# aim-uofa/GenPercept

Hardware: AMD Instinct MI355X
Metric: images/sec at 768x768 bf16 (depth) (higher is better)
Workload: dtype bf16; 1 GPU; depth head, SD2.1 VAE-enc + UNet(t=1) + VAE-dec, 768x768, batch 4/GPU (BASELINE.json configs[1]); global_batch=4, resolution=768, parallelism=dp1 (batch-sharded, weights replicated, no data-path collective), weights=random-init SD2.1 architecture (865.9M + 83.7M params)

## Files before the change

genpercept_amd/csrc/attention.hip:

```cpp
#include <cstdlib>

#include "common.h"
#include "kernels.h"

GP_DEV int attn_off128(int row, int slot) { return row * 128 + ((slot ^ ((row >> 1) & 7)) << 4); }

#ifndef GP_FLASH_DEFER
#define GP_FLASH_DEFER 0.f
#endif
template <int NKB>
__global__ __launch_bounds__(256, 2) void flash_attn64_kernel(const h16_t* __restrict__ Q, const h16_t* __restrict__ K,
                                                            const h16_t* __restrict__ Vt, h16_t* __restrict__ O, int T, int heads, int ldq,
                                                            int ldk, int Tpad, int ldo) {
    constexpr int KEYS = 32 * NKB, KBYTES = KEYS * 128, NH = NKB / 2;
    constexpr int STAGE = 2 * KBYTES;
    extern __shared__ __attribute__((aligned(16))) char smem[];
    const int tid = threadIdx.x, lane = tid & 63;
    const int wave = __builtin_amdgcn_readfirstlane(tid >> 6);
    const int nqb = (T + 127) >> 7;
    const int sid = xcd_remap(blockIdx.x, gridDim.x);
    const int qb = sid % nqb, bh = sid / nqb;
    const int h = bh % heads, b = bh / heads;
    const int q0 = qb * 128 + wave * 32;
    const int l31 = lane & 31, hh = lane >> 5;

    const h16_t* Qb = Q + (long long)b * T * ldq + h * 64;
    const h16_t* Kb = K + (long long)b * T * ldk + h * 64;
    const h16_t* Vb = Vt + ((long long)b * heads + h) * 64 * Tpad;

    h16x8_t qf[4];
    {
        const int q = q0 + l31;
        const bool ok = q < T;
#pragma unroll
        for (int ks = 0; ks < 4; ++ks) {
            if (ok) qf[ks] = *(const h16x8_t*)(Qb + (long long)q * ldq + ks * 16 + hh * 8);
            else qf[ks] = h16x8_t{0, 0, 0, 0, 0, 0, 0, 0};
        }
    }

    const int chunk = (lane & 7) ^ ((wave * 4 + (lane >> 4)) & 7);
    const int nt = (T + KEYS - 1) / KEYS;
    const buf_rsrc_t k_rs = make_rsrc(Kb, (unsigned)(((long long)T - 1) * ldk * 2 + 128));
    const buf_rsrc_t v_rs = make_rsrc(Vb, (unsigned)(64ll * Tpad * 2));
    const unsigned k_lane = (unsigned)(((lane >> 3) & 3) + 8 * (lane >> 5)) * (unsigned)(ldk * 2) + chunk * 16;
    const unsigned v_lane = ((unsigned)(lane >> 3) * Tpad + chunk * 8) * 2;
    auto stage = [&](int buf, int kt) {
        char* sb = smem + buf * STAGE;
#pragma unroll
        for (int i = 0; i < NKB; ++i) {
            const int g = wave + 4 * i;
            blds16(k_rs, k_lane, (unsigned)(kt * KEYS + (g >> 1) * 16 + 4 * (g & 1)) * (unsigned)(ldk * 2), sb + g * 1024);
        }
#pragma unroll
        for (int hf = 0; hf < NH; ++hf)
#pragma unroll
            for (int i = 0; i < 2; ++i) {
                const int k0 = kt * KEYS + hf * 64;
                const unsigned so = k0 < Tpad ? (unsigned)((wave + 4 * i) * 8 * Tpad + k0) * 2u : 0xfffff000u;
                blds16(v_rs, v_lane, so, sb + KBYTES + hf * 8192 + (wave + 4 * i) * 1024);
            }
    };

    f32x16_t o_acc[2];
#pragma unroll
    for (int d = 0; d < 2; ++d)
#pragma unroll
        for (int r = 0; r < 16; ++r) o_acc[d][r] = 0.f;
    float m_run = -1e30f;
    float l_run = 0.f;
    const float sc = 0.125f * 1.44269504088896340736f;
    f32x16_t zero16;
#pragma unroll
    for (int r = 0; r < 16; ++r) zero16[r] = 0.f;
    int cur = 0;
    const unsigned smem_base = (unsigned)(unsigned long long)smem;

    auto tile = [&](int kt, auto maskc) __attribute__((always_inline)) {
        constexpr bool MASK = decltype(maskc)::value != 0;
        const unsigned sb = smem_base + cur * STAGE;
        f32x16_t s_acc[NKB];
#pragma unroll
        for (int kb = 0; kb < NKB; ++kb) {
            const int row = kb * 32 + l31;
#pragma unroll
            for (int ks = 0; ks < 4; ++ks) {
                const h16x8_t kf = lds_frag(sb + attn_off128(row, ks * 2 + hh), 0);
                s_acc[kb] = mfma_32x32x16(kf, qf[ks], ks == 0 ? zero16 : s_acc[kb]);
            }
        }
        if (MASK) {
            const int kbase = kt * KEYS + 8 * hh;
#pragma unroll
            for (int kb = 0; kb < NKB; ++kb)
#pragma unroll
                for (int r = 0; r < 16; ++r)
                    if (kbase + kb * 32 + (r & 7) + 16 * (r >> 3) >= T) s_acc[kb][r] = -1e30f;
        }
        float mx = s_acc[0][0];
#pragma unroll
        for (int kb = 0; kb < NKB; ++kb)
#pragma unroll
            for (int r = 0; r < 16; ++r) mx = fmaxf(mx, s_acc[kb][r]);
        mx = xor32_max(mx);
        if (__builtin_amdgcn_ballot_w64((mx - m_run) * sc > GP_FLASH_DEFER) != 0ull) {
            const float m_new = fmaxf(m_run, mx);
            const float alpha = __builtin_amdgcn_exp2f((m_run - m_new) * sc);
            m_run = m_new;
            l_run *= alpha;
#pragma unroll
            for (int d = 0; d < 2; ++d)
#pragma unroll
                for (int r = 0; r < 16; ++r) o_acc[d][r] *= alpha;
        }
        typedef float f32x2_t __attribute__((ext_vector_type(2)));
        const f32x2_t sc2 = {sc, sc}, nm2 = {-m_run * sc, -m_run * sc};
        f32x2_t rs2 = {0.f, 0.f};
#pragma unroll
        for (int kb = 0; kb < NKB; ++kb)
#pragma unroll
            for (int r = 0; r < 16; r += 2) {
                f32x2_t t = {s_acc[kb][r], s_acc[kb][r + 1]};
                t = __builtin_elementwise_fma(t, sc2, nm2);
                t.x = __builtin_amdgcn_exp2f(t.x);
                t.y = __builtin_amdgcn_exp2f(t.y);
                s_acc[kb][r] = t.x;
                s_acc[kb][r + 1] = t.y;
                rs2 += t;
            }
        l_run += rs2.x + rs2.y;
#pragma unroll
        for (int kb = 0; kb < NKB; ++kb)
#pragma unroll
            for (int j = 0; j < 2; ++j) {
                union { h16x8_t v; unsigned u[4]; } pf;
#pragma unroll
                for (int e = 0; e < 4; ++e) pf.u[e] = pack_h16x2_ns(s_acc[kb][8 * j + 2 * e], s_acc[kb][8 * j + 2 * e + 1]);
                const int slot = (kb & 1) * 4 + 2 * j + hh;
#pragma unroll
                for (int d = 0; d < 2; ++d) {
                    const h16x8_t vf = lds_frag(sb + KBYTES + (kb >> 1) * 8192 + attn_off128(d * 32 + l31, slot), 0);
                    o_acc[d] = mfma_32x32x16(vf, pf.v, o_acc[d]);
                }
            }
    };

#pragma unroll
    for (int s0 = 0; s0 < 1; ++s0)
        if (s0 < nt) stage(s0, s0);
    int nxt = 1;
    auto step = [&](int kt, auto maskc) __attribute__((always_inline)) {
        wait_vm<0>();
        __builtin_amdgcn_s_barrier();
        if (kt + 1 < nt) stage(nxt, kt + 1);
        tile(kt, maskc);
        cur = cur + 1 == 2 ? 0 : cur + 1;
        nxt = nxt + 1 == 2 ? 0 : nxt + 1;
    };
    const bool ragged = nt * KEYS > T;
    const int nfull = ragged ? nt - 1 : nt;
    for (int kt = 0; kt < nfull; ++kt) step(kt, IC<0>{});
    if (ragged) step(nt - 1, IC<1>{});
    l_run += __shfl_xor(l_run, 32);
    const float inv = 1.f / l_run;
    const int q = q0 + l31;
    if (q < T) {
        h16_t* ob = O + ((long long)b * T + q) * ldo + h * 64;
#pragma unroll
        for (int d = 0; d < 2; ++d)
#pragma unroll
            for (int g = 0; g < 4; ++g) {
                const uint2 pk = pack_h16x4(o_acc[d][4 * g] * inv, o_acc[d][4 * g + 1] * inv, o_acc[d][4 * g + 2] * inv, o_acc[d][4 * g + 3] * inv);
                *(uint2*)(ob + d * 32 + 8 * g + 4 * hh) = pk;
            }
    }
}

void launch_flash_attn64(const h16_t* q, const h16_t* k, const h16_t* vt, h16_t* out, int B, int T, int heads,
                         int ldq, int ldk, int Tpad, int ldo, hipStream_t s) {
    dim3 grid(((T + 127) / 128) * heads * B);
    hipLaunchKernelGGL(flash_attn64_kernel<2>, grid, dim3(256), 2 * 16384, s, q, k, vt, out, T, heads, ldq, ldk, Tpad, ldo);
}

__global__ __launch_bounds__(256, 2) void flash_attn64_split_kernel(const h16_t* __restrict__ QKhi, const h16_t* __restrict__ QKlo,
                                                                  const h16_t* __restrict__ Vthi, const h16_t* __restrict__ Vtlo,
                                                                  h16_t* __restrict__ O, int T, int heads, int ld, int Tpad) {
    constexpr int KEYS = 64, KBYTES = 8192, STAGE = 4 * KBYTES;
    extern __shared__ __attribute__((aligned(16))) char smem[];
    const int tid = threadIdx.x, lane = tid & 63;
    const int wave = __builtin_amdgcn_readfirstlane(tid >> 6);
    const int nqb = (T + 127) >> 7;
    const int sid = xcd_remap(blockIdx.x, gridDim.x);
    const int qb = sid % nqb, bh = sid / nqb;
    const int h = bh % heads, b = bh / heads;
    const int C = heads * 64;
    const int q0 = qb * 128 + wave * 32;
    const int l31 = lane & 31, hh = lane >> 5;

    const long long qoff = (long long)b * T * ld + h * 64;
    const long long voff = ((long long)b * heads + h) * 64 * Tpad;
    h16x8_t qh[4], ql[4];
    {
        const int q = q0 + l31;
        const bool ok = q < T;
#pragma unroll
        for (int ks = 0; ks < 4; ++ks) {
            if (ok) {
                qh[ks] = *(const h16x8_t*)(QKhi + qoff + (long long)q * ld + ks * 16 + hh * 8);
                ql[ks] = *(const h16x8_t*)(QKlo + qoff + (long long)q * ld + ks * 16 + hh * 8);
            } else {
                qh[ks] = ql[ks] = h16x8_t{0, 0, 0, 0, 0, 0, 0, 0};
            }
        }
    }
    const int chunk = (lane & 7) ^ ((wave * 4 + (lane >> 4)) & 7);
    const int nt = (T + KEYS - 1) / KEYS;
    const unsigned kbytes = (unsigned)(((long long)T - 1) * ld * 2 + 128);
    const buf_rsrc_t kh_rs = make_rsrc(QKhi + qoff + C, kbytes), kl_rs = make_rsrc(QKlo + qoff + C, kbytes);
    const buf_rsrc_t vh_rs = make_rsrc(Vthi + voff, (unsigned)(64ll * Tpad * 2)), vl_rs = make_rsrc(Vtlo + voff, (unsigned)(64ll * Tpad * 2));
    const unsigned k_lane = (unsigned)(((lane >> 3) & 3) + 8 * (lane >> 5)) * (unsigned)(ld * 2) + chunk * 16;
    const unsigned v_lane = ((unsigned)(lane >> 3) * Tpad + chunk * 8) * 2;
    auto stage = [&](int buf, int kt) {
        char* sb = smem + buf * STAGE;
#pragma unroll
        for (int i = 0; i < 2; ++i) {
            const int g = wave + 4 * i;
            const unsigned ko = (unsigned)(kt * KEYS + (g >> 1) * 16 + 4 * (g & 1)) * (unsigned)(ld * 2);
            blds16(kh_rs, k_lane, ko, sb + g * 1024);
            blds16(kl_rs, k_lane, ko, sb + KBYTES + g * 1024);
            const int k0 = kt * KEYS;
            const unsigned so = k0 < Tpad ? (unsigned)((wave + 4 * i) * 8 * Tpad + k0) * 2u : 0xfffff000u;
            blds16(vh_rs, v_lane, so, sb + 2 * KBYTES + g * 1024);
            blds16(vl_rs, v_lane, so, sb + 3 * KBYTES + g * 1024);
        }
    };
    f32x16_t o_acc[2];
#pragma unroll
    for (int d = 0; d < 2; ++d)
#pragma unroll
        for (int r = 0; r < 16; ++r) o_acc[d][r] = 0.f;
    float m_run = -1e30f, l_run = 0.f;
    const float sc = 0.125f * 1.44269504088896340736f;
    f32x16_t zero16;
#pragma unroll
    for (int r = 0; r < 16; ++r) zero16[r] = 0.f;
    int cur = 0;
    const unsigned smem_base = (unsigned)(unsigned long long)smem;

    auto tile = [&](int kt, auto maskc) __attribute__((always_inline)) {
        constexpr bool MASK = decltype(maskc)::value != 0;
        const unsigned sb = smem_base + cur * STAGE;
        f32x16_t s_acc[2];
#pragma unroll
        for (int kb = 0; kb < 2; ++kb) {
            const int row = kb * 32 + l31;
#pragma unroll
            for (int ks = 0; ks < 4; ++ks) {
                const h16x8_t kfh = lds_frag(sb + attn_off128(row, ks * 2 + hh), 0);
                const h16x8_t kfl = lds_frag(sb + KBYTES + attn_off128(row, ks * 2 + hh), 0);
                s_acc[kb] = mfma_32x32x16(kfl, qh[ks], ks == 0 ? zero16 : s_acc[kb]);
                s_acc[kb] = mfma_32x32x16(kfh, ql[ks], s_acc[kb]);
                s_acc[kb] = mfma_32x32x16(kfh, qh[ks], s_acc[kb]);
            }
        }
        if (MASK) {
            const int kbase = kt * KEYS + 8 * hh;
#pragma unroll
            for (int kb = 0; kb < 2; ++kb)
#pragma unroll
                for (int r = 0; r < 16; ++r)
                    if (kbase + kb * 32 + (r & 7) + 16 * (r >> 3) >= T) s_acc[kb][r] = -1e30f;
        }
        float mx = s_acc[0][0];
#pragma unroll
        for (int kb = 0; kb < 2; ++kb)
#pragma unroll
            for (int r = 0; r < 16; ++r) mx = fmaxf(mx, s_acc[kb][r]);
        mx = xor32_max(mx);
        if (__builtin_amdgcn_ballot_w64(mx > m_run) != 0ull) {
            const float m_new = fmaxf(m_run, mx);
            const float alpha = __builtin_amdgcn_exp2f((m_run - m_new) * sc);
            m_run = m_new;
            l_run *= alpha;
#pragma unroll
            for (int d = 0; d < 2; ++d)
#pragma unroll
                for (int r = 0; r < 16; ++r) o_acc[d][r] *= alpha;
        }
        const float nm = -m_run * sc;
        float rs = 0.f;
#pragma unroll
        for (int kb = 0; kb < 2; ++kb)
#pragma unroll
            for (int r = 0; r < 16; ++r) {
                const float t = __builtin_amdgcn_exp2f(__builtin_fmaf(s_acc[kb][r], sc, nm));
                s_acc[kb][r] = t;
                rs += t;
            }
        l_run += rs;
#pragma unroll
        for (int kb = 0; kb < 2; ++kb)
#pragma unroll
            for (int j = 0; j < 2; ++j) {
                union { h16x8_t v; unsigned u[4]; } ph, pl;
#pragma unroll
                for (int e = 0; e < 4; ++e) {
                    const float a = s_acc[kb][8 * j + 2 * e], c = s_acc[kb][8 * j + 2 * e + 1];
                    ph.u[e] = pack_h16x2_ns(a, c);
                    pl.u[e] = pack_h16x2_ns(a - h16_lo(ph.u[e]), c - h16_hi(ph.u[e]));
                }
                const int slot = kb * 4 + 2 * j + hh;
#pragma unroll
                for (int d = 0; d < 2; ++d) {
                    const h16x8_t vfh = lds_frag(sb + 2 * KBYTES + attn_off128(d * 32 + l31, slot), 0);
                    const h16x8_t vfl = lds_frag(sb + 3 * KBYTES + attn_off128(d * 32 + l31, slot), 0);
                    o_acc[d] = mfma_32x32x16(vfl, ph.v, o_acc[d]);
                    o_acc[d] = mfma_32x32x16(vfh, pl.v, o_acc[d]);
                    o_acc[d] = mfma_32x32x16(vfh, ph.v, o_acc[d]);
                }
            }
    };
    stage(0, 0);
    auto step = [&](int kt, auto maskc) __attribute__((always_inline)) {
        wait_vm<0>();
        __builtin_amdgcn_s_barrier();
        if (kt + 1 < nt) stage(cur ^ 1, kt + 1);
        tile(kt, maskc);
        cur ^= 1;
    };
    const bool ragged = nt * KEYS > T;
    const int nfull = ragged ? nt - 1 : nt;
    for (int kt = 0; kt < nfull; ++kt) step(kt, IC<0>{});
    if (ragged) step(nt - 1, IC<1>{});
    l_run += __shfl_xor(l_run, 32);
    const float inv = 1.f / l_run;
    const int q = q0 + l31;
    if (q < T) {
        h16_t* ob = O + ((long long)b * T + q) * 3 * C + h * 64;
#pragma unroll
        for (int d = 0; d < 2; ++d)
#pragma unroll
            for (int g = 0; g < 4; ++g) {
                const float v0 = o_acc[d][4 * g] * inv, v1 = o_acc[d][4 * g + 1] * inv, v2 = o_acc[d][4 * g + 2] * inv, v3 = o_acc[d][4 * g + 3] * inv;
                const unsigned h0 = pack_h16x2(v0, v1), h1 = pack_h16x2(v2, v3);
                const unsigned l0 = pack_h16x2(v0 - h16_lo(h0), v1 - h16_hi(h0)), l1 = pack_h16x2(v2 - h16_lo(h1), v3 - h16_hi(h1));
                const int c = d * 32 + 8 * g + 4 * hh;
                *(uint2*)(ob + c) = make_uint2(h0, h1);
                *(uint2*)(ob + C + c) = make_uint2(l0, l1);
                *(uint2*)(ob + 2 * C + c) = make_uint2(h0, h1);
            }
    }
}
void launch_flash_attn64_split(const h16_t* qk_hi, const h16_t* qk_lo, const h16_t* vt_hi, const h16_t* vt_lo, h16_t* out, int B, int T, int heads, int ld,
                               int Tpad, hipStream_t s) {
    static unsigned long long attr_mask = 0;
    gp_once_per_device(&attr_mask, [&] {
        (void)hipFuncSetAttribute((const void*)flash_attn64_split_kernel, hipFuncAttributeMaxDynamicSharedMemorySize, 2 * 32768);
    });
    dim3 grid(((T + 127) / 128) * heads * B);
    hipLaunchKernelGGL(flash_attn64_split_kernel, grid, dim3(256), 2 * 32768, s, qk_hi, qk_lo, vt_hi, vt_lo, out, T, heads, ld, Tpad);
}

constexpr int F5_KBYTES = 32 * 1024;
constexpr int F5_QV = 24;
constexpr int F5_RD = 6;
constexpr int F5_LDS = 4 * F5_KBYTES + 4 * (32 - F5_QV) * 1024;
typedef __attribute__((address_space(3))) h16x8_t* lds_frag_wptr;
GP_DEV float other_half(float v) {
    typedef unsigned u32x2p_t __attribute__((ext_vector_type(2)));
    const u32x2p_t r = __builtin_amdgcn_permlane32_swap(__float_as_uint(v), __float_as_uint(v), false, false);
    return (threadIdx.x & 32) ? __uint_as_float(r[0]) : __uint_as_float(r[1]);
}
GP_DEV int k512_off(int row, int slot) { return row * 1024 + ((slot ^ (row & 15)) << 4); }
GP_DEV int v512_off(int row, int slot) { return row * 64 + ((slot ^ ((row >> 2) & 3)) << 4); }
GP_DEV int pi23(int i) { return (i & ~12) | ((i & 4) << 1) | ((i & 8) >> 1); }

__global__ __launch_bounds__(256) void flash_attn512_kernel(const h16_t* __restrict__ Q, const h16_t* __restrict__ K,
                                                             const h16_t* __restrict__ Vt, h16_t* __restrict__ O,
                                                             float* __restrict__ part_o,
                                                             float* __restrict__ part_ml, int B, int T, int ldq, int ldk, int Tpad, int ldo,
                                                             float scale) {
    extern __shared__ __attribute__((aligned(16))) char smem[];
    const int tid = threadIdx.x, lane = tid & 63;
    const int wave = __builtin_amdgcn_readfirstlane(tid >> 6);
    const int l31 = lane & 31, hh = lane >> 5;
    const int nqb = (T + 127) >> 7, nblocks = B * nqb, G = gridDim.x;
    const int nt = (T + 31) >> 5;
    const int rounds = nblocks / G, L = nblocks - rounds * G, S = L ? G / L : 0;
    const int sid = xcd_remap(blockIdx.x, G);
    const unsigned smem_base = (unsigned)(unsigned long long)smem;
    const float sc = scale * 1.44269504088896340736f;
    f32x16_t zero16;
#pragma unroll
    for (int r = 0; r < 16; ++r) zero16[r] = 0.f;

    const int items = rounds + ((L && sid / S < L) ? 1 : 0);
    for (int it = 0; it < items; ++it) {
        const bool whole = it < rounds;
        const int part = whole ? 0 : sid % S;
        const int t0 = whole ? 0 : (int)((long long)nt * part / S), t1 = whole ? nt : (int)((long long)nt * (part + 1) / S);
        const int Li = (L % B == 0) ? L / B : 0;
        int b, qb;
        if (whole) {
            const int w = it * G + sid, per = nqb - Li;
            b = Li ? w / per : w / nqb;
            qb = Li ? w - b * per : w - b * nqb;
        } else {
            const int lb = sid / S;
            b = Li ? lb / Li : (rounds * G + lb) / nqb;
            qb = Li ? nqb - Li + (lb - b * Li) : rounds * G + lb - b * nqb;
        }
        const int q0 = qb * 128 + wave * 32;
        const h16_t* Qb = Q + (long long)b * T * ldq;
        const h16_t* Kb = K + (long long)b * T * ldk;
        const h16_t* Vb = Vt + (long long)b * 512 * Tpad;

        __syncthreads();
        h16x8_t qf[F5_QV];
        const unsigned q_lds = smem_base + 4 * F5_KBYTES + wave * ((32 - F5_QV) * 1024) + lane * 16;
        {
            const int q = q0 + l31;
            const bool ok = q < T;
#pragma unroll
            for (int ks = 0; ks < 32; ++ks) {
                h16x8_t v = h16x8_t{0, 0, 0, 0, 0, 0, 0, 0};
                if (ok) v = *(const h16x8_t*)(Qb + (long long)q * ldq + ks * 16 + hh * 8);
                if ((ks & 3) != 3) qf[3 * (ks >> 2) + (ks & 3)] = v;
                else *(lds_frag_wptr)(q_lds + (ks >> 2) * 1024) = v;
            }
            asm volatile("" ::"v"(qf[F5_QV - 1]));
        }
        const buf_rsrc_t k_rs = make_rsrc(Kb, (unsigned)((long long)T * ldk * 2));
        const buf_rsrc_t v_rs = make_rsrc(Vb, (unsigned)(512ll * Tpad * 2));
        unsigned koff[8];
#pragma unroll
        for (int n = 0; n < 8; ++n) koff[n] = (unsigned)(lane ^ ((wave & 1) * 8 + n)) << 4;
        const unsigned v_lane_off = ((unsigned)(lane >> 2) * Tpad + (((lane & 3) ^ ((lane >> 4) & 3)) << 3)) * 2;
        auto stage_piece = [&](int slot, int kt, int pc) __attribute__((always_inline)) {
            char* sb = smem + slot * F5_KBYTES;
            if (pc < 8) {
                const int i = wave * 8 + pc;
                const int key = min(kt * 32 + pi23(i), T - 1);
                blds16(k_rs, koff[pc & 7], (unsigned)key * (unsigned)(ldk * 2), sb + i * 1024);
            } else {
                const int m = pc - 8;
                blds16(v_rs, v_lane_off, (unsigned)((128 * wave + 16 * m) * Tpad + kt * 32) * 2u, sb + 2 * F5_KBYTES + (wave * 8 + m) * 1024);
            }
        };
        auto stage = [&](int slot, int kt) __attribute__((always_inline)) {
#pragma unroll
            for (int pc = 0; pc < 16; ++pc) stage_piece(slot, kt, pc);
        };

        f32x16_t o_acc[16];
#pragma unroll
        for (int d = 0; d < 16; ++d) o_acc[d] = zero16;
        float m_run = -1e30f, l_run = 0.f, alpha = 1.f;
        const unsigned ka0 = l31 * 1024 + ((hh ^ (l31 & 15)) << 4);
        unsigned va[2];
#pragma unroll
        for (int j = 0; j < 2; ++j) va[j] = 2 * F5_KBYTES + l31 * 64 + (((2 * j + hh) ^ ((l31 >> 2) & 3)) << 4);

        h16x8_t pf[2];
        auto s_phase = [&](unsigned sb, int kt, bool do_stage, int slot_next, auto maskc) __attribute__((always_inline)) -> bool {
            constexpr bool MASK = decltype(maskc)::value != 0;
            f32x16_t s0, s1;
            h16x8_t fr[F5_RD], ql[2];
            auto rd = [&](int ks) __attribute__((always_inline)) {
                fr[ks % F5_RD] = lds_frag(sb + (ka0 ^ ((ks & 7) << 5)), (ks >> 3) * 256);
                if ((ks & 3) == 3) ql[(ks >> 2) & 1] = lds_frag(q_lds, (ks >> 2) * 1024);
            };
#pragma unroll
            for (int ks = 0; ks < F5_RD; ++ks) rd(ks);
#pragma unroll
            for (int ks = 0; ks < 32; ++ks) {
                const h16x8_t qv = (ks & 3) != 3 ? qf[3 * (ks >> 2) + ((ks & 3) != 3 ? (ks & 3) : 0)] : ql[(ks >> 2) & 1];
                if (ks & 1) s1 = mfma_32x32x16(fr[ks % F5_RD], qv, ks == 1 ? zero16 : s1);
                else s0 = mfma_32x32x16(fr[ks % F5_RD], qv, ks == 0 ? zero16 : s0);
                if (ks + F5_RD < 32) rd(ks + F5_RD);
                if (do_stage && (ks & 1)) stage_piece(slot_next, kt + 1, ks >> 1);
            }
            f32x16_t s_acc;
#pragma unroll
            for (int r = 0; r < 16; ++r) s_acc[r] = s0[r] + s1[r];
            if (MASK) {
                const int kbase = kt * 32 + 8 * hh;
#pragma unroll
                for (int r = 0; r < 16; ++r)
                    if (kbase + (r & 7) + 16 * (r >> 3) >= T) s_acc[r] = -1e30f;
            }
            float mx = s_acc[0];
#pragma unroll
            for (int r = 1; r < 16; ++r) mx = fmaxf(mx, s_acc[r]);
            mx = fmaxf(mx, other_half(mx));
            const bool moved = __builtin_amdgcn_ballot_w64((mx - m_run) * sc > 8.f) != 0ull;
            if (moved) {
                const float m_new = fmaxf(m_run, mx);
                alpha = __builtin_amdgcn_exp2f((m_run - m_new) * sc);
                m_run = m_new;
                l_run *= alpha;
            }
            const float nm = -m_run * sc;
            float rs = 0.f;
#pragma unroll
            for (int r = 0; r < 16; ++r) {
                s_acc[r] = __builtin_amdgcn_exp2f(__builtin_fmaf(s_acc[r], sc, nm));
                rs += s_acc[r];
            }
            l_run += rs;
#pragma unroll
            for (int j = 0; j < 2; ++j) {
                union { h16x8_t v; unsigned u[4]; } t;
#pragma unroll
                for (int e = 0; e < 4; ++e) t.u[e] = pack_h16x2_ns(s_acc[8 * j + 2 * e], s_acc[8 * j + 2 * e + 1]);
                pf[j] = t.v;
            }
            return moved;
        };
        auto pv_phase = [&](unsigned sb) __attribute__((always_inline)) {
            h16x8_t fr[F5_RD];
            auto rd = [&](int st) __attribute__((always_inline)) { fr[st % F5_RD] = lds_frag(sb + va[st >> 4], (st & 15) * 2048); };
#pragma unroll
            for (int st = 0; st < F5_RD; ++st) rd(st);
#pragma unroll
            for (int st = 0; st < 32; ++st) {
                o_acc[st & 15] = mfma_32x32x16(fr[st % F5_RD], pf[st >> 4], o_acc[st & 15]);
                if (st + F5_RD < 32) rd(st + F5_RD);
            }
        };

        if (t0 < t1) stage(0, t0);
        __builtin_amdgcn_s_waitcnt(0x0070);
        int kt = t0;
        for (;;) {
            bool pending = false;
            unsigned sb = 0;
            for (; kt < t1; ++kt) {
                const int rel = (kt - t0) & 1;
                sb = smem_base + rel * F5_KBYTES;
                wait_vm<0>();
                __builtin_amdgcn_s_barrier();
                const bool nx = kt + 1 < t1;
                const bool moved = (kt * 32 + 32 > T) ? s_phase(sb, kt, nx, rel ^ 1, IC<1>{}) : s_phase(sb, kt, nx, rel ^ 1, IC<0>{});
                if (moved) { pending = true; break; }
                pv_phase(sb);
            }
            if (!pending) break;
#pragma unroll
            for (int d = 0; d < 16; ++d) {
#pragma unroll
                for (int r = 0; r < 16; ++r) o_acc[d][r] *= alpha;
                __builtin_amdgcn_sched_barrier(0);
            }
            pv_phase(sb);
            ++kt;
            __builtin_amdgcn_s_waitcnt(0x0070);
        }
        l_run += other_half(l_run);
        const int q = q0 + l31;
        if (whole) {
            const float inv = 1.f / l_run;
            if (q < T) {
                h16_t* ob = O + ((long long)b * T + q) * ldo;
#pragma unroll
                for (int d = 0; d < 16; ++d)
#pragma unroll
                    for (int g = 0; g < 4; ++g) {
                        const uint2 pk = pack_h16x4(o_acc[d][4 * g] * inv, o_acc[d][4 * g + 1] * inv, o_acc[d][4 * g + 2] * inv, o_acc[d][4 * g + 3] * inv);
                        *(uint2*)(ob + d * 32 + 8 * g + 4 * hh) = pk;
                    }
            }
        } else {
            const long long slot = (long long)(sid / S) * S + part;
            float* po = part_o + (slot * 128 + wave * 32 + l31) * 512;
#pragma unroll
            for (int d = 0; d < 16; ++d)
#pragma unroll
                for (int g = 0; g < 4; ++g)
                    *(float4*)(po + d * 32 + 8 * g + 4 * hh) = float4{o_acc[d][4 * g], o_acc[d][4 * g + 1], o_acc[d][4 * g + 2], o_acc[d][4 * g + 3]};
            if (hh == 0) {
                float* pm = part_ml + (slot * 128 + wave * 32 + l31) * 2;
                pm[0] = m_run;
                pm[1] = l_run;
            }
        }
    }
}

__global__ __launch_bounds__(256) void flash512_combine_kernel(const float* __restrict__ part_o, const float* __restrict__ part_ml,
                                                                h16_t* __restrict__ O, int T, int nqb, int first_blk, int Li, int S, int ldo,
                                                                float scale) {
    const int lb = blockIdx.x >> 2, qq = (blockIdx.x & 3) * 32 + (threadIdx.x >> 3);
    const int b = Li ? lb / Li : (first_blk + lb) / nqb;
    const int q = (Li ? nqb - Li + (lb - b * Li) : first_blk + lb - b * nqb) * 128 + qq;
    if (q >= T) return;
    const float sc = scale * 1.44269504088896340736f;
    float m = -1e30f;
    for (int p = 0; p < S; ++p) m = fmaxf(m, part_ml[(((long long)lb * S + p) * 128 + qq) * 2]);
    float l = 0.f;
    float acc[64];
#pragma unroll
    for (int i = 0; i < 64; ++i) acc[i] = 0.f;
    const int c0 = (threadIdx.x & 7) * 4;
    for (int p = 0; p < S; ++p) {
        const long long row = ((long long)lb * S + p) * 128 + qq;
        const float w = __builtin_amdgcn_exp2f((part_ml[row * 2] - m) * sc);
        l += w * part_ml[row * 2 + 1];
        const float* po = part_o + row * 512 + c0;
#pragma unroll
        for (int i = 0; i < 16; ++i) {
            const float4 v = *(const float4*)(po + 32 * i);
            acc[4 * i] += w * v.x; acc[4 * i + 1] += w * v.y; acc[4 * i + 2] += w * v.z; acc[4 * i + 3] += w * v.w;
        }
    }
    const float inv = 1.f / l;
    h16_t* ob = O + ((long long)b * T + q) * ldo + c0;
#pragma unroll
    for (int i = 0; i < 16; ++i)
        *(uint2*)(ob + 32 * i) = pack_h16x4(acc[4 * i] * inv, acc[4 * i + 1] * inv, acc[4 * i + 2] * inv, acc[4 * i + 3] * inv);
}

bool flash_attn512_supported(int C) { return C == 512 && !gp_sw().no_flash512; }
static int flash512_grid(int nblocks, int ncu, int T) {
    if (nblocks >= ncu) return ncu;
    const int nt = (T + 31) / 32;
    int parts = ncu / nblocks;
    if (parts > nt / 8) parts = nt / 8;
    return parts >= 2 ? parts * nblocks : nblocks;
}
long long flash_attn512_workspace_floats(int B, int T, int ncu) {
    const int nblocks = B * ((T + 127) / 128), G = flash512_grid(nblocks, ncu, T);
    const int L = nblocks % G;
    return L ? (long long)(G / L) * L * 128 * (512 + 2) : 0;
}
void launch_flash_attn512(const h16_t* q, const h16_t* k, const h16_t* vt, h16_t* out, float* ws, int B, int T, int ldq,
                          int ldk, int Tpad, int ldo, float scale, int ncu, hipStream_t s) {
    static unsigned long long attr_mask = 0;
    gp_once_per_device(&attr_mask, [&] { (void)hipFuncSetAttribute((const void*)flash_attn512_kernel, hipFuncAttributeMaxDynamicSharedMemorySize, F5_LDS); });
    const int nqb = (T + 127) / 128, nblocks = B * nqb, G = flash512_grid(nblocks, ncu, T);
    const int rounds = nblocks / G, L = nblocks - rounds * G, S = L ? G / L : 0;
    float* part_o = ws;
    float* part_ml = ws ? ws + (long long)S * L * 128 * 512 : nullptr;
    hipLaunchKernelGGL(flash_attn512_kernel, dim3(G), dim3(256), F5_LDS, s, q, k, vt, out, part_o, part_ml, B, T, ldq, ldk, Tpad, ldo,
                       scale);
    if (L) hipLaunchKernelGGL(flash512_combine_kernel, dim3(L * 4), dim3(256), 0, s, part_o, part_ml, out, T, nqb, rounds * G, (L % B == 0) ? L / B : 0,
                              S, ldo, scale);
}

__global__ __launch_bounds__(256) void cross_attn_small_kernel(const h16_t* __restrict__ q, const float* __restrict__ kc,
                                                                const float* __restrict__ vc, h16_t* __restrict__ out, long long nrh,
                                                                int C, int heads, int L) {
    const long long idx = (long long)blockIdx.x * 256 + threadIdx.x;
    if (idx >= nrh) return;
    const long long row = idx / heads;
    const int h = (int)(idx - row * heads);
    float qv[64];
    const h16_t* qp = q + row * C + h * 64;
#pragma unroll
    for (int i = 0; i < 8; ++i) {
        const uint4 raw = *(const uint4*)(qp + i * 8);
        const unsigned w[4] = {raw.x, raw.y, raw.z, raw.w};
#pragma unroll
        for (int k = 0; k < 4; ++k) { qv[i * 8 + 2 * k] = h16_lo(w[k]); qv[i * 8 + 2 * k + 1] = h16_hi(w[k]); }
    }
    float o[64];
#pragma unroll
    for (int d = 0; d < 64; ++d) o[d] = 0.f;
    float m = -1e30f, l = 0.f;
    for (int j = 0; j < L; ++j) {
        const float* kp = kc + (long long)j * C + h * 64;
        float s = 0.f;
#pragma unroll
        for (int d = 0; d < 64; ++d) s += qv[d] * kp[d];
        s *= 0.125f;
        const float mn = fmaxf(m, s);
        const float a = __expf(m - mn), pj = __expf(s - mn);
        m = mn;
        l = l * a + pj;
        const float* vp = vc + (long long)j * C + h * 64;
#pragma unroll
        for (int d = 0; d < 64; ++d) o[d] = o[d] * a + pj * vp[d];
    }
    const float inv = 1.f / l;
    h16_t* op = out + row * C + h * 64;
#pragma unroll
    for (int i = 0; i < 8; ++i) {
        uint4 r;
        r.x = pack_h16x2(o[i * 8] * inv, o[i * 8 + 1] * inv);
        r.y = pack_h16x2(o[i * 8 + 2] * inv, o[i * 8 + 3] * inv);
        r.z = pack_h16x2(o[i * 8 + 4] * inv, o[i * 8 + 5] * inv);
        r.w = pack_h16x2(o[i * 8 + 6] * inv, o[i * 8 + 7] * inv);
        *(uint4*)(op + i * 8) = r;
    }
}

void launch_cross_attn_small(const h16_t* q, const float* kc, const float* vc, h16_t* out, int rows, int C, int L, hipStream_t s) {
    const int heads = C / 64;
    const long long nrh = (long long)rows * heads;
    hipLaunchKernelGGL(cross_attn_small_kernel, dim3((unsigned)((nrh + 255) / 256)), dim3(256), 0, s, q, kc, vc, out, nrh, C, heads, L);
}

__global__ __launch_bounds__(256) void softmax_rows_kernel(const float* __restrict__ in, h16_t* __restrict__ out, int T, int ld, float scale) {
    __shared__ float red[8];
    const long long row = blockIdx.x;
    const float* x = in + row * ld;
    h16_t* y = out + row * ld;
    const int tid = threadIdx.x, lane = tid & 63, wv = tid >> 6;
    const float sc = scale * 1.44269504088896340736f;
    float mx = -1e30f;
    for (int i = tid; i < T; i += 256) mx = fmaxf(mx, x[i] * sc);
#pragma unroll
    for (int o = 32; o > 0; o >>= 1) mx = fmaxf(mx, __shfl_xor(mx, o));
    if (lane == 0) red[wv] = mx;
    __syncthreads();
    mx = fmaxf(fmaxf(red[0], red[1]), fmaxf(red[2], red[3]));
    float sum = 0.f;
    for (int i = tid; i < T; i += 256) sum += exp2f(x[i] * sc - mx);
#pragma unroll
    for (int o = 32; o > 0; o >>= 1) sum += __shfl_xor(sum, o);
    if (lane == 0) red[4 + wv] = sum;
    __syncthreads();
    const float inv = 1.f / (red[4] + red[5] + red[6] + red[7]);
    for (int i = tid; i < ld; i += 256) y[i] = i < T ? f_to_h16(exp2f(x[i] * sc - mx) * inv) : (h16_t)0;
}

GP_DEV float4 load4(const float* p, int i) { return ((const float4*)p)[i]; }
GP_DEV float4 load4(const _Float16* p, int i) {
    typedef _Float16 h4_t __attribute__((ext_vector_type(4)));
    const h4_t h = ((const h4_t*)p)[i];
    return make_float4((float)h[0], (float)h[1], (float)h[2], (float)h[3]);
}
template <int NV, typename TIN>
__global__ __launch_bounds__(256) void softmax_rows_reg_kernel(const TIN* __restrict__ in, h16_t* __restrict__ out, int T, int ld, float scale) {
    __shared__ float red[8];
    const long long row = blockIdx.x;
    const TIN* x = in + row * ld;
    uint2* y = (uint2*)(out + row * ld);
    const int tid = threadIdx.x, lane = tid & 63, wv = tid >> 6;
    const float sc = scale * 1.44269504088896340736f;
    const int nvec = ld >> 2;
    float4 v[NV];
    float mx = -1e30f;
#pragma unroll
    for (int k = 0; k < NV; ++k) {
        const int i = k * 256 + tid;
        v[k] = i < nvec ? load4(x, i) : make_float4(0.f, 0.f, 0.f, 0.f);
        const int e0 = i * 4;
        v[k].x = e0 + 0 < T ? v[k].x : -1e30f;
        v[k].y = e0 + 1 < T ? v[k].y : -1e30f;
        v[k].z = e0 + 2 < T ? v[k].z : -1e30f;
        v[k].w = e0 + 3 < T ? v[k].w : -1e30f;
        mx = fmaxf(mx, fmaxf(fmaxf(v[k].x, v[k].y), fmaxf(v[k].z, v[k].w)));
    }
#pragma unroll
    for (int o = 32; o > 0; o >>= 1) mx = fmaxf(mx, __shfl_xor(mx, o));
    if (lane == 0) red[wv] = mx;
    __syncthreads();
    mx = fmaxf(fmaxf(red[0], red[1]), fmaxf(red[2], red[3]));
    const float nm = -mx * sc;
    float sum = 0.f;
#pragma unroll
    for (int k = 0; k < NV; ++k) {
        v[k].x = __builtin_amdgcn_exp2f(__builtin_fmaf(v[k].x, sc, nm));
        v[k].y = __builtin_amdgcn_exp2f(__builtin_fmaf(v[k].y, sc, nm));
        v[k].z = __builtin_amdgcn_exp2f(__builtin_fmaf(v[k].z, sc, nm));
        v[k].w = __builtin_amdgcn_exp2f(__builtin_fmaf(v[k].w, sc, nm));
        sum += (v[k].x + v[k].y) + (v[k].z + v[k].w);
    }
#pragma unroll
    for (int o = 32; o > 0; o >>= 1) sum += __shfl_xor(sum, o);
    if (lane == 0) red[4 + wv] = sum;
    __syncthreads();
    const float inv = 1.f / (red[4] + red[5] + red[6] + red[7]);
#pragma unroll
    for (int k = 0; k < NV; ++k) {
        const int i = k * 256 + tid;
        if (i < nvec) y[i] = pack_h16x4(v[k].x * inv, v[k].y * inv, v[k].z * inv, v[k].w * inv);
    }
}

void launch_softmax_rows(const float* in, h16_t* out, int rows, int T, int ld, float scale, hipStream_t s) {
    if ((ld & 3) == 0 && scale > 0.f && ld <= 16384) {
        if (ld <= 4096) hipLaunchKernelGGL((softmax_rows_reg_kernel<4, float>), dim3(rows), dim3(256), 0, s, in, out, T, ld, scale);
        else if (ld <= 9216) hipLaunchKernelGGL((softmax_rows_reg_kernel<9, float>), dim3(rows), dim3(256), 0, s, in, out, T, ld, scale);
        else hipLaunchKernelGGL((softmax_rows_reg_kernel<16, float>), dim3(rows), dim3(256), 0, s, in, out, T, ld, scale);
        return;
    }
    hipLaunchKernelGGL(softmax_rows_kernel, dim3(rows), dim3(256), 0, s, in, out, T, ld, scale);
}

bool softmax_rows_f16_supported(int ld) { return (ld & 3) == 0 && ld <= 16384; }
void launch_softmax_rows_f16(const void* in, h16_t* out, int rows, int T, int ld, float scale, hipStream_t s) {
    const _Float16* x = (const _Float16*)in;
    if (ld <= 4096) hipLaunchKernelGGL((softmax_rows_reg_kernel<4, _Float16>), dim3(rows), dim3(256), 0, s, x, out, T, ld, scale);
    else if (ld <= 9216) hipLaunchKernelGGL((softmax_rows_reg_kernel<9, _Float16>), dim3(rows), dim3(256), 0, s, x, out, T, ld, scale);
    else hipLaunchKernelGGL((softmax_rows_reg_kernel<16, _Float16>), dim3(rows), dim3(256), 0, s, x, out, T, ld, scale);
}

GP_SAT_TU(attention)
```

Before: 93.74 images/sec.

## Pin flash-attn512 output accumulator in AGPRs via inline-asm MFMA

Rewrites the head-dim-512 flash attention kernel so the 256-float output accumulator lives in the accumulation registers, driven by hand-written inline-asm MFMA, zero, rescale and readout routines. The goal is to stop the compiler from spilling or shuffling the large accumulator between VGPRs and AGPRs. It also hoists the first V-fragment LDS reads into the end of the QK phase, and replaces the conditional staging branch with a zero-size buffer resource so the out-of-range loads become no-ops. Q loads are made unconditional with clamped rows. The cost is fragile manual hazard handling with s_nop padding and switch-based register indexing, which the compiler can no longer schedule around.

```diff
diff --git a/genpercept_amd/csrc/attention.hip b/genpercept_amd/csrc/attention.hip
--- a/genpercept_amd/csrc/attention.hip
+++ b/genpercept_amd/csrc/attention.hip
@@ -371,6 +371,47 @@
     const u32x2p_t r = __builtin_amdgcn_permlane32_swap(__float_as_uint(v), __float_as_uint(v), false, false);
     return (threadIdx.x & 32) ? __uint_as_float(r[0]) : __uint_as_float(r[1]);
 }
+#if GP_F16
+#define F5_MFMA "v_mfma_f32_32x32x16_f16"
+#else
+#define F5_MFMA "v_mfma_f32_32x32x16_bf16"
+#endif
+GP_DEV void f5_mfma_first(f32x16_t& c, h16x8_t a, h16x8_t b) { asm volatile(F5_MFMA " %0, %1, %2, 0" : "=&v"(c) : "v"(a), "v"(b)); }
+GP_DEV void f5_mfma_acc(f32x16_t& c, h16x8_t a, h16x8_t b) { asm volatile(F5_MFMA " %0, %1, %2, %0" : "+v"(c) : "v"(a), "v"(b)); }
+GP_DEV void f5_mfma_settle(f32x16_t& c0, f32x16_t& c1) { asm volatile("s_nop 15\n\ts_nop 3" : "+v"(c0), "+v"(c1)); }
+#define F5_A10(t) "a" #t "0", "a" #t "1", "a" #t "2", "a" #t "3", "a" #t "4", "a" #t "5", "a" #t "6", "a" #t "7", "a" #t "8", "a" #t "9"
+#define F5_ALL_ACC                                                                                                                            \
+    F5_A10(), F5_A10(1), F5_A10(2), F5_A10(3), F5_A10(4), F5_A10(5), F5_A10(6), F5_A10(7), F5_A10(8), F5_A10(9), F5_A10(10), F5_A10(11),     \
+        F5_A10(12), F5_A10(13), F5_A10(14), F5_A10(15), F5_A10(16), F5_A10(17), F5_A10(18), F5_A10(19), F5_A10(20), F5_A10(21), F5_A10(22),  \
+        F5_A10(23), F5_A10(24), "a250", "a251", "a252", "a253", "a254", "a255"
+GP_DEV void f5_acc_zero() {
+    asm volatile(".set f5_i, 0\n\t.rept 256\n\tv_accvgpr_write_b32 a[f5_i], 0\n\t.set f5_i, f5_i + 1\n\t.endr" ::: F5_ALL_ACC);
+}
+GP_DEV void f5_acc_scale(float alpha) {
+    float t;
+    asm volatile(".set f5_i, 0\n\t.rept 256\n\tv_accvgpr_read_b32 %0, a[f5_i]\n\tv_mul_f32 %0, %1, %0\n\tv_accvgpr_write_b32 a[f5_i], %0\n\t"
+                 ".set f5_i, f5_i + 1\n\t.endr\n\ts_nop 7"
+                 : "=&v"(t) : "v"(alpha) : F5_ALL_ACC);
+}
+#define F5_PV(d) case d: asm volatile(F5_MFMA " a[" #d "*16:" #d "*16+15], %0, %1, a[" #d "*16:" #d "*16+15]" ::"v"(a), "v"(b)); break;
+GP_DEV void f5_acc_mfma(int d, h16x8_t a, h16x8_t b) {
+    switch (d) { F5_PV(0) F5_PV(1) F5_PV(2) F5_PV(3) F5_PV(4) F5_PV(5) F5_PV(6) F5_PV(7) F5_PV(8) F5_PV(9) F5_PV(10) F5_PV(11) F5_PV(12) F5_PV(13) F5_PV(14) F5_PV(15) }
+}
+#undef F5_PV
+GP_DEV void f5_acc_settle() { asm volatile("s_nop 15\n\ts_nop 3"); }
+#define F5_RDL(d, r) "v_accvgpr_read_b32 %" #r ", a[" #d "*16+" #r "]\n\t"
+#define F5_GET(d)                                                                                                                              \
+    case d:                                                                                                                                    \
+        asm volatile(F5_RDL(d, 0) F5_RDL(d, 1) F5_RDL(d, 2) F5_RDL(d, 3) F5_RDL(d, 4) F5_RDL(d, 5) F5_RDL(d, 6) F5_RDL(d, 7) F5_RDL(d, 8)       \
+                         F5_RDL(d, 9) F5_RDL(d, 10) F5_RDL(d, 11) F5_RDL(d, 12) F5_RDL(d, 13) F5_RDL(d, 14) F5_RDL(d, 15)                       \
+                     : "=v"(t[0]), "=v"(t[1]), "=v"(t[2]), "=v"(t[3]), "=v"(t[4]), "=v"(t[5]), "=v"(t[6]), "=v"(t[7]), "=v"(t[8]), "=v"(t[9]),  \
+                       "=v"(t[10]), "=v"(t[11]), "=v"(t[12]), "=v"(t[13]), "=v"(t[14]), "=v"(t[15]));                                           \
+        break;
+GP_DEV void f5_acc_get(int d, float* t) {
+    switch (d) { F5_GET(0) F5_GET(1) F5_GET(2) F5_GET(3) F5_GET(4) F5_GET(5) F5_GET(6) F5_GET(7) F5_GET(8) F5_GET(9) F5_GET(10) F5_GET(11) F5_GET(12) F5_GET(13) F5_GET(14) F5_GET(15) }
+}
+#undef F5_GET
+#undef F5_RDL
 GP_DEV int k512_off(int row, int slot) { return row * 1024 + ((slot ^ (row & 15)) << 4); }
 GP_DEV int v512_off(int row, int slot) { return row * 64 + ((slot ^ ((row >> 2) & 3)) << 4); }
 GP_DEV int pi23(int i) { return (i & ~12) | ((i & 4) << 1) | ((i & 8) >> 1); }
@@ -390,9 +431,6 @@
     const int sid = xcd_remap(blockIdx.x, G);
     const unsigned smem_base = (unsigned)(unsigned long long)smem;
     const float sc = scale * 1.44269504088896340736f;
-    f32x16_t zero16;
-#pragma unroll
-    for (int r = 0; r < 16; ++r) zero16[r] = 0.f;
 
     const int items = rounds + ((L && sid / S < L) ? 1 : 0);
     for (int it = 0; it < items; ++it) {
@@ -421,17 +459,19 @@
         {
             const int q = q0 + l31;
             const bool ok = q < T;
+            const h16_t* qrow = Qb + (long long)min(q, T - 1) * ldq + hh * 8;
 #pragma unroll
             for (int ks = 0; ks < 32; ++ks) {
-                h16x8_t v = h16x8_t{0, 0, 0, 0, 0, 0, 0, 0};
-                if (ok) v = *(const h16x8_t*)(Qb + (long long)q * ldq + ks * 16 + hh * 8);
+                h16x8_t v = *(const h16x8_t*)(qrow + ks * 16);
+                if (!ok) v = h16x8_t{0, 0, 0, 0, 0, 0, 0, 0};
                 if ((ks & 3) != 3) qf[3 * (ks >> 2) + (ks & 3)] = v;
                 else *(lds_frag_wptr)(q_lds + (ks >> 2) * 1024) = v;
             }
             asm volatile("" ::"v"(qf[F5_QV - 1]));
         }
-        const buf_rsrc_t k_rs = make_rsrc(Kb, (unsigned)((long long)T * ldk * 2));
-        const buf_rsrc_t v_rs = make_rsrc(Vb, (unsigned)(512ll * Tpad * 2));
+        const unsigned k_bytes = (unsigned)((long long)T * ldk * 2), v_bytes = (unsigned)(512ll * Tpad * 2);
+        buf_rsrc_t k_rs = make_rsrc(Kb, k_bytes);
+        buf_rsrc_t v_rs = make_rsrc(Vb, v_bytes);
         unsigned koff[8];
 #pragma unroll
         for (int n = 0; n < 8; ++n) koff[n] = (unsigned)(lane ^ ((wave & 1) * 8 + n)) << 4;
@@ -452,20 +492,22 @@
             for (int pc = 0; pc < 16; ++pc) stage_piece(slot, kt, pc);
         };
 
-        f32x16_t o_acc[16];
-#pragma unroll
-        for (int d = 0; d < 16; ++d) o_acc[d] = zero16;
+        f5_acc_zero();
         float m_run = -1e30f, l_run = 0.f, alpha = 1.f;
         const unsigned ka0 = l31 * 1024 + ((hh ^ (l31 & 15)) << 4);
         unsigned va[2];
 #pragma unroll
         for (int j = 0; j < 2; ++j) va[j] = 2 * F5_KBYTES + l31 * 64 + (((2 * j + hh) ^ ((l31 >> 2) & 3)) << 4);
 
-        h16x8_t pf[2];
+        h16x8_t pf[2], vfr[F5_RD];
+        unsigned sb = 0;
+        auto rd_v = [&](int st) __attribute__((always_inline)) { vfr[st % F5_RD] = lds_frag(sb + va[st >> 4], (st & 15) * 2048); };
         auto s_phase = [&](unsigned sb, int kt, bool do_stage, int slot_next, auto maskc) __attribute__((always_inline)) -> bool {
             constexpr bool MASK = decltype(maskc)::value != 0;
             f32x16_t s0, s1;
             h16x8_t fr[F5_RD], ql[2];
+            k_rs = make_rsrc(Kb, do_stage ? k_bytes : 0u);
+            v_rs = make_rsrc(Vb, do_stage ? v_bytes : 0u);
             auto rd = [&](int ks) __attribute__((always_inline)) {
                 fr[ks % F5_RD] = lds_frag(sb + (ka0 ^ ((ks & 7) << 5)), (ks >> 3) * 256);
                 if ((ks & 3) == 3) ql[(ks >> 2) & 1] = lds_frag(q_lds, (ks >> 2) * 1024);
@@ -475,11 +517,15 @@
 #pragma unroll
             for (int ks = 0; ks < 32; ++ks) {
                 const h16x8_t qv = (ks & 3) != 3 ? qf[3 * (ks >> 2) + ((ks & 3) != 3 ? (ks & 3) : 0)] : ql[(ks >> 2) & 1];
-                if (ks & 1) s1 = mfma_32x32x16(fr[ks % F5_RD], qv, ks == 1 ? zero16 : s1);
-                else s0 = mfma_32x32x16(fr[ks % F5_RD], qv, ks == 0 ? zero16 : s0);
+                if (ks < 2) f5_mfma_first(ks ? s1 : s0, fr[ks % F5_RD], qv);
+                else f5_mfma_acc((ks & 1) ? s1 : s0, fr[ks % F5_RD], qv);
                 if (ks + F5_RD < 32) rd(ks + F5_RD);
-                if (do_stage && (ks & 1)) stage_piece(slot_next, kt + 1, ks >> 1);
-            }
+                if (ks & 1) stage_piece(slot_next, kt + 1, ks >> 1);
+            }
+#pragma unroll
+            for (int st = 0; st < F5_RD; ++st) rd_v(st);
+            f5_mfma_settle(s0, s1);
+            __builtin_amdgcn_sched_barrier(0);
             f32x16_t s_acc;
 #pragma unroll
             for (int r = 0; r < 16; ++r) s_acc[r] = s0[r] + s1[r];
@@ -517,15 +563,12 @@
             }
             return moved;
         };
-        auto pv_phase = [&](unsigned sb) __attribute__((always_inline)) {
-            h16x8_t fr[F5_RD];
-            auto rd = [&](int st) __attribute__((always_inline)) { fr[st % F5_RD] = lds_frag(sb + va[st >> 4], (st & 15) * 2048); };
-#pragma unroll
-            for (int st = 0; st < F5_RD; ++st) rd(st);
+        auto pv_phase = [&](unsigned) __attribute__((always_inline)) {
+            asm volatile("s_nop 1");
 #pragma unroll
             for (int st = 0; st < 32; ++st) {
-                o_acc[st & 15] = mfma_32x32x16(fr[st % F5_RD], pf[st >> 4], o_acc[st & 15]);
-                if (st + F5_RD < 32) rd(st + F5_RD);
+                f5_acc_mfma(st & 15, vfr[st % F5_RD], pf[st >> 4]);
+                if (st + F5_RD < 32) rd_v(st + F5_RD);
             }
         };
 
@@ -534,7 +577,6 @@
         int kt = t0;
         for (;;) {
             bool pending = false;
-            unsigned sb = 0;
             for (; kt < t1; ++kt) {
                 const int rel = (kt - t0) & 1;
                 sb = smem_base + rel * F5_KBYTES;
@@ -546,38 +588,42 @@
                 pv_phase(sb);
             }
             if (!pending) break;
-#pragma unroll
-            for (int d = 0; d < 16; ++d) {
-#pragma unroll
-                for (int r = 0; r < 16; ++r) o_acc[d][r] *= alpha;
-                __builtin_amdgcn_sched_barrier(0);
-            }
+            f5_acc_scale(alpha);
             pv_phase(sb);
             ++kt;
             __builtin_amdgcn_s_waitcnt(0x0070);
         }
+        wait_vm<0>();
         l_run += other_half(l_run);
         const int q = q0 + l31;
+        f5_acc_settle();
+        int l31_o = l31, hh_o = hh;
+        asm volatile("" : "+v"(l31_o), "+v"(hh_o));
         if (whole) {
             const float inv = 1.f / l_run;
             if (q < T) {
-                h16_t* ob = O + ((long long)b * T + q) * ldo;
-#pragma unroll
-                for (int d = 0; d < 16; ++d)
+                h16_t* ob = O + ((long long)b * T + q0) * ldo + (unsigned)(l31_o * ldo);
+#pragma unroll
+                for (int d = 0; d < 16; ++d) {
+                    float o[16];
+                    f5_acc_get(d, o);
 #pragma unroll
                     for (int g = 0; g < 4; ++g) {
-                        const uint2 pk = pack_h16x4(o_acc[d][4 * g] * inv, o_acc[d][4 * g + 1] * inv, o_acc[d][4 * g + 2] * inv, o_acc[d][4 * g + 3] * inv);
-                        *(uint2*)(ob + d * 32 + 8 * g + 4 * hh) = pk;
+                        const uint2 pk = pack_h16x4(o[4 * g] * inv, o[4 * g + 1] * inv, o[4 * g + 2] * inv, o[4 * g + 3] * inv);
+                        *(uint2*)(ob + d * 32 + 8 * g + 4 * hh_o) = pk;
                     }
+                }
             }
         } else {
             const long long slot = (long long)(sid / S) * S + part;
-            float* po = part_o + (slot * 128 + wave * 32 + l31) * 512;
-#pragma unroll
-            for (int d = 0; d < 16; ++d)
-#pragma unroll
-                for (int g = 0; g < 4; ++g)
-                    *(float4*)(po + d * 32 + 8 * g + 4 * hh) = float4{o_acc[d][4 * g], o_acc[d][4 * g + 1], o_acc[d][4 * g + 2], o_acc[d][4 * g + 3]};
+            float* po = part_o + (slot * 128 + wave * 32 + l31_o) * 512;
+#pragma unroll
+            for (int d = 0; d < 16; ++d) {
+                float o[16];
+                f5_acc_get(d, o);
+#pragma unroll
+                for (int g = 0; g < 4; ++g) *(float4*)(po + d * 32 + 8 * g + 4 * hh_o) = float4{o[4 * g], o[4 * g + 1], o[4 * g + 2], o[4 * g + 3]};
+            }
             if (hh == 0) {
                 float* pm = part_ml + (slot * 128 + wave * 32 + l31) * 2;
                 pm[0] = m_run;
```

New measurement: 94.74 images/sec (median of 6 runs). 1.1% higher.
